# svg-project/Sparse-VideoGen

Measured on AMD Instinct MI355X. Metric: attn_tflops_svg1_block_sparse, higher is better.
Workload: dtype bf16; 1 GPU; HunyuanVideo T2V hy720p SVG1 sparse layer-call: sample_mse(64 rows) + band attention with fused head placement, cfg=1 H=24 D=128 F=33 P=3600 ctx=256 prompt=64 S=119056 band=15616 density=0.2456; parallelism=single, variant=0, heads=alt

## Files before the change

include/svg_attn.h:

```cpp
#ifndef SVG_ATTN_H_
#define SVG_ATTN_H_

#include <stddef.h>
#include <stdint.h>

#ifdef __cplusplus
extern "C" {
#endif

#define SVG_DTYPE_BF16 0
#define SVG_DTYPE_F16 1
#define SVG_DTYPE_F32 2

#define SVG_OK 0
#define SVG_ERR_BAD_ARG (-1)
#define SVG_ERR_UNSUPPORTED (-2)
#define SVG_ERR_WORKSPACE (-3)
#define SVG_ERR_LAUNCH (-4)

#define SVG_ABI_VERSION 4
int svg_abi_version(void);

const char* svg_strerror(int code);
int svg_last_hip_error(void);
// ... 239 lines not shown
                              float sm_scale, const svg_band_mask_t* masks, const svg_band_mask_t* alt_masks,
                              const int32_t* group_heads, int32_t n_groups, const svg_perm_desc_t* perm,
                              const int32_t* use_alt_flag, int32_t q_prescaled, const svg_attn_layout_t* layout, void* stream);

size_t svg_band_attention_fp8_workspace_bytes(int32_t BH, int32_t S, int32_t D);
int svg_band_attention_fp8(const void* q, const void* k, const void* v, void* o, int32_t BH, int32_t S, int32_t D, int32_t dtype,
                           float sm_scale, const svg_band_mask_t* mask, const svg_perm_desc_t* perm, void* workspace,
                           size_t workspace_bytes, void* stream);
int svg_band_attention_fp8_stage(const void* q, const void* k, const void* v, void* o, int32_t BH, int32_t S, int32_t D, int32_t dtype,
                                 float sm_scale, const svg_band_mask_t* mask, const svg_perm_desc_t* perm, void* workspace,
                                 size_t workspace_bytes, int32_t stage, void* stream);

size_t svg_varblock_attention_fp8_workspace_bytes(int32_t Hq, int32_t Hkv, int32_t QB, int32_t KB, int32_t Sq, int32_t Skv, int32_t D);
int svg_varblock_attention_fp8(const void* q, const void* k, const void* v, void* o, int32_t Hq, int32_t Hkv, int32_t Sq, int32_t Skv,
                               int32_t D, int32_t dtype, float sm_scale, const uint8_t* block_map, const int32_t* q_sizes,
                               const int32_t* k_sizes, int32_t QB, int32_t KB, const int32_t* q_row_idx, const int32_t* kv_row_idx,
                               void* workspace, size_t workspace_bytes, void* stream);

int32_t svg_band_attention_notify_target(int32_t S, const svg_band_mask_t* mask);
int svg_band_attention_notify(const void* q, const void* k, const void* v, void* o, int32_t BH, int32_t S, int32_t D,
                              int32_t dtype, float sm_scale, const svg_band_mask_t* mask, const svg_perm_desc_t* perm,
                              int32_t* done_per_head, int32_t done_words, void* stream);
int svg_wait_counters(const int32_t* counters, int32_t n, int32_t target, void* stream);
int svg_wait_counters_deadline(const int32_t* counters, int32_t n, int32_t target, int32_t timeout_ms, int32_t* timed_out,
                               void* stream);
int32_t svg_band_attention_notify_layout(int32_t S, const svg_band_mask_t* mask, int32_t nseg, int32_t* row_bounds, int32_t* targets);
int svg_band_attention_notify_seg(const void* q, const void* k, const void* v, void* o, int32_t BH, int32_t S, int32_t D,
                                  int32_t dtype, float sm_scale, const svg_band_mask_t* mask, const svg_perm_desc_t* perm,
                                  int32_t* done, int32_t done_words, int32_t nseg, void* stream);
int svg_band_attention_prescaled_notify_seg(const void* q_scaled, const void* k, const void* v, void* o, int32_t BH, int32_t S,
                                            int32_t D, int32_t dtype, const svg_band_mask_t* mask, const svg_perm_desc_t* perm,
                                            int32_t* done, int32_t done_words, int32_t nseg, void* stream);

int32_t svg_band_queue_order(int32_t BH, int32_t S, const svg_band_mask_t* mask, int32_t* out, int32_t out_words);
int svg_debug_band_queue_cap(int32_t max_workgroups);
int64_t svg_debug_band_replays(int32_t reset);
int32_t svg_debug_band_row_cursor(int32_t S, int32_t vid0, int32_t num_frame, int32_t frame_size, int32_t token_major,
                                  const int32_t* k0, int32_t n, int32_t* out, int32_t out_words, int32_t* cheap);

int svg_debug_pp_trace(uint64_t* out104);

int svg_debug_clock_probe(const int32_t* stop_flag, uint64_t* out2, int32_t max_ms, void* stream);

int svg_debug_wg_trace(uint64_t* out, int32_t n_workgroups);

#ifdef __cplusplus
}
#endif

#include "svg_attn_sparse_lse.h"
#include "svg_attn_f32_parts.h"
#include "svg_attn_band_lse_forms.h"
#include "svg_attn_band_window.h"
#include "svg_attn_band_shard.h"
#include "svg_attn_band_shard_switch.h"
#include "svg_attn_profile_shard.h"
#endif
```

sparse-videogen_amd/csrc/attention.hip:

```cpp
#include <algorithm>
#include <atomic>
#include <mutex>

#include "attn_core.h"
#include "attn_m16.h"
#include "band_policy.h"

namespace svg {

template <typename T, int D, int NW>
__global__ __launch_bounds__(NW * 64, 2) void band_attn_kernel(typename BandPolicy<T, D, NW>::Params prm) {
    extern __shared__ __attribute__((aligned(16))) char smem[];
    attn_body<T, D, NW, BandPolicy<T, D, NW>>(prm, smem, nullptr);
}

template <typename T, int D>
__global__ __launch_bounds__(512, (D == 64 ? 4 : 2)) void band_attn_pp2_kernel(typename BandPolicy<T, D, 8>::Params prm) {
    extern __shared__ __attribute__((aligned(16))) char smem[];
    attn_body_pp2<T, D, BandPolicy<T, D, 8>, false, 0, false, D == 64>(prm, smem, nullptr);
}
template <typename T>
__global__ __launch_bounds__(512, 4) void band_attn_pp2_switch64_kernel(typename BandPolicy<T, 64, 8>::Params prm,
                                                                        typename BandPolicy<T, 64, 8>::Params prm_alt,
                                                                        const int32_t* __restrict__ flag) {
// ... 912 lines not shown
extern "C" int64_t svg_debug_band_replays(int32_t reset) {
    unsigned n = 0;
    if (hipDeviceSynchronize() != hipSuccess || hipMemcpyFromSymbol(&n, HIP_SYMBOL(g_band_replays), sizeof n) != hipSuccess) return -1;
    const unsigned zero = 0;
    if (reset && hipMemcpyToSymbol(HIP_SYMBOL(g_band_replays), &zero, sizeof zero) != hipSuccess) return -1;
    return (int64_t)n;
}

extern "C" int32_t svg_debug_band_row_cursor(int32_t S, int32_t vid0, int32_t num_frame, int32_t frame_size, int32_t token_major,
                                             const int32_t* k0, int32_t n, int32_t* out, int32_t out_words, int32_t* cheap) {
    using Pol = svg::BandPolicy<__bf16, 128, 8>;
    if (S <= 0 || n < 0 || !k0 || !out || (int64_t)out_words < (int64_t)n * kBN) return -1;
    const svg_band_mask_t mask{S, S, 0, 0, 0, 0};
    const int64_t flag = 1;
    const svg_perm_desc_t perm{&flag, vid0, num_frame, frame_size};
    if (check_band_mask(S, &mask, &perm) != SVG_OK) return -1;
    const Pol::Params p = svg::make_band_params<Pol, __bf16>(nullptr, nullptr, nullptr, nullptr, 1, S, 1.f, &mask, &perm);
    Pol::Ctx c{};
    c.perm = token_major != 0;
    for (int row = 0; row < kBN; ++row) {
        Pol::RowWalk w;
        Pol::row_walk_init(p, c, w);
        int phys = 0;
        for (int i = 0; i < n; ++i) {
            Pol::RowWalk probe = w;
            if (cheap) cheap[i] = Pol::row_walk_cheap(probe, k0[i]) ? 1 : 0;
            Pol::row_walk_next(p, w, phys, k0[i], row);
            out[(size_t)i * kBN + row] = phys;
        }
    }
    return n;
}

extern "C" int svg_debug_wg_trace(uint64_t* out, int n_workgroups) { return g_trace_reader(out, true, n_workgroups); }
extern "C" int svg_debug_pp_trace(uint64_t* out104) { return g_trace_reader(out104, false, 0); }
```

sparse-videogen_amd/csrc/attn_m16.h:

```cpp
#pragma once
#include "attn_core.h"

namespace svg {

template <typename T>
struct Mfma16;
template <>
struct Mfma16<__bf16> {
    static __device__ __forceinline__ f32x4 mfma(bf16x8 a, bf16x8 b, f32x4 c) { return __builtin_amdgcn_mfma_f32_16x16x32_bf16(a, b, c, 0, 0, 0); }
    static __device__ __forceinline__ f32x4 mfma_keep_c(bf16x8 a, bf16x8 b, const f32x4& c) {
        f32x4 d;
        asm volatile("v_mfma_f32_16x16x32_bf16 %0, %1, %2, %3" : "=&v"(d) : "v"(a), "v"(b), "v"(c));
        return d;
    }
};
template <>
struct Mfma16<_Float16> {
    static __device__ __forceinline__ f32x4 mfma(f16x8 a, f16x8 b, f32x4 c) { return __builtin_amdgcn_mfma_f32_16x16x32_f16(a, b, c, 0, 0, 0); }
    static __device__ __forceinline__ f32x4 mfma_keep_c(f16x8 a, f16x8 b, const f32x4& c) {
        f32x4 d;
        asm volatile("v_mfma_f32_16x16x32_f16 %0, %1, %2, %3" : "=&v"(d) : "v"(a), "v"(b), "v"(c));
        return d;
    }
};
// ... 53 lines not shown
struct HasRowO32<P, std::void_t<decltype(&P::o32_base)>> : std::true_type {};
template <typename T, typename E>
__device__ __forceinline__ f32x4 o32_values(const f32x4& acc, float inv) {
    f32x4 o4;
    if constexpr (std::is_same_v<T, _Float16>) {
        typename E::v4 h4;
#pragma unroll
        for (int j = 0; j < 4; ++j) h4[j] = E::from_float(acc[j] * inv);
        u32x2 hb = __builtin_bit_cast(u32x2, h4);
        asm("" : "+v"(hb));
        h4 = __builtin_bit_cast(typename E::v4, hb);
#pragma unroll
        for (int j = 0; j < 4; ++j) {
            float a = acc[j];
            asm("" : "+v"(a));
            float p = a * inv;
            asm("" : "+v"(p));
            const float h = (float)h4[j];
            if ((float)(_Float16)p != h)
                p = __uint_as_float(fabsf(h) > fabsf(p) ? __float_as_uint(p) + 1u : __float_as_uint(p) - 1u);
            o4[j] = p;
        }
    } else {
#pragma unroll
        for (int j = 0; j < 4; ++j) o4[j] = acc[j] * inv;
    }
    return o4;
}

template <typename P, typename = void>
struct HasRowCursor : std::false_type {};
template <typename P>
struct HasRowCursor<P, std::void_t<decltype(P::kRowCursor)>> : std::true_type {};

template <bool when_set>
__device__ __forceinline__ void pp_barrier_sel(int flag) {
    __builtin_amdgcn_sched_barrier(0);
    if constexpr (when_set) asm volatile("s_cmp_eq_u32 %0, 0\n\ts_cbranch_scc1 1f\n\ts_waitcnt lgkmcnt(0)\n\ts_barrier\n1:" ::"s"(flag) : "memory", "scc");
    else asm volatile("s_cmp_lg_u32 %0, 0\n\ts_cbranch_scc1 1f\n\ts_waitcnt lgkmcnt(0)\n\ts_barrier\n1:" ::"s"(flag) : "memory", "scc");
    __builtin_amdgcn_sched_barrier(0);
}

template <typename T>
__device__ __forceinline__ u32x2 add_rounded16(u32x2 a, u32x2 b) {
    using E = Elt<T>;
    const typename E::v4 x = __builtin_bit_cast(typename E::v4, a), y = __builtin_bit_cast(typename E::v4, b);
    typename E::v4 s;
#pragma unroll
    for (int j = 0; j < 4; ++j) s[j] = E::from_float(E::to_float(x[j]) + E::to_float(y[j]));
    return __builtin_bit_cast(u32x2, s);
}

constexpr int kCheckEvery = 8;
template <typename T, typename P, bool TRACE = false, int ONEBAR = -1, bool PRE = false, bool SPEC = false>
__device__ __forceinline__ bool attn_m16_tile(const typename P::Params& prm, const typename P::Ctx& ctx, char* smem,
                                              int check_mask = kCheckEvery - 1, unsigned* replay_ctr = nullptr) {
    using E = Elt<T>;
    using M = Mfma16<T>;
    using V8 = typename E::v8;
    constexpr int D = 128;
    constexpr int NW = 8;
    constexpr int KS = D / 32;
    constexpr int NDB = D / 16;
    using Img = KvImage16<D>;
    constexpr int NS = 4;
    constexpr int kImg = Img::kImg, kStage = Img::kStage;
// ... 44 lines not shown
    int nphys = 0, nnext = 0;
    unsigned req_ko = 0, req_vo = 0;
    auto resolve = [&](int t, auto guard_c) {
        if constexpr (kCursor) {
            if (!decltype(guard_c)::value || t < nT) P::row_walk_next(prm, cur, nnext, P::tile_key0(ctx, t), krow);
        } else if constexpr (decltype(guard_c)::value) {
            nnext = (t < nT) ? P::kv_phys(prm, ctx, cur, t, krow) : 0;
        } else {
            nnext = P::kv_phys(prm, ctx, cur, t, krow);
        }
    };
    constexpr std::true_type kGuarded{};
    auto take = [&]() {
        if constexpr (kCursor) {
            req_ko = __umul24((unsigned)nnext, k_rsb) + col_v;
            req_vo = __umul24((unsigned)nnext, v_rsb) + col_v;
            asm volatile("" : "+v"(req_ko), "+v"(req_vo));
        } else {
            nphys = nnext;
        }
    };
    auto dma_piece = [&](int t, auto j_c) {
        constexpr int j = decltype(j_c)::value;
        const unsigned st = __builtin_amdgcn_readfirstlane(lds_piece + (unsigned)((t % NS) * kStage) + j * (kBN * 64));
        const unsigned ko = kCursor ? req_ko : __umul24((unsigned)nphys, k_rsb) + col_v;
        const unsigned vo = kCursor ? req_vo : __umul24((unsigned)nphys, v_rsb) + col_v;
        lds_dma16_kv<kImg>(st, ko, vo, (const char*)kb_ + j * 64, (const char*)vb + j * 64);
    };
    auto dma_issue = [&](int t) {
        dma_piece(t, std::integral_constant<int, 0>{});
        dma_piece(t, std::integral_constant<int, 1>{});
    };
    const int dist = lagging ? 3 : 2;
    for (int t = 0; t < dist; ++t) {
        resolve(t, kGuarded);
        take();
        if (t < nT) dma_issue(t);
    }
    resolve(dist, kGuarded);

    int q_log[2];
    V8 qf[2][KS];
    int m_a0[2], m_b0[2];
    unsigned m_alen[2], m_blen[2];
#pragma unroll
    for (int rb = 0; rb < 2; ++rb) {
        const int row_in_wg = wave * 32 + rb * 16 + n16;
        const int qp = P::q_phys(prm, ctx, row_in_wg);
        q_log[rb] = P::q_logical(ctx, row_in_wg);
        const T* qrow = qb + (size_t)(qp >= 0 ? qp : 0) * P::q_rs(prm) + g4 * 8;
#pragma unroll
        for (int ks = 0; ks < KS; ++ks) qf[rb][ks] = *(const V8*)(qrow + ks * 32);
        P::row_intervals(prm, ctx, q_log[rb], m_a0[rb], m_alen[rb], m_b0[rb], m_blen[rb]);
    }

    const int k_lane = Img::k_lane(g4, n16);
    const int v_lane0 = Img::v_lane0(g4, n16);
    const int v_lane1 = v_lane0 ^ 32;

    float m_run[2] = {-INFINITY, -INFINITY}, m_use[2] = {0.f, 0.f}, l_run[2] = {0.f, 0.f}, psum[2] = {0.f, 0.f};
    float m_sub[2] = {kBias, kBias};
    f32x4 acc_l[2] = {{0.f, 0.f, 0.f, 0.f}, {0.f, 0.f, 0.f, 0.f}};
    V8 ones8;
#pragma unroll
    for (int j = 0; j < 8; ++j) ones8[j] = E::from_float(1.f);
    bool force_exact = true;
// ... 37 lines not shown
    float psum_thr = -1.f;

    auto kfrag = [&](const char* st, int kblk, int ks) -> i16x8 { return Img::kfrag(st, k_lane, kblk, ks); };
    auto vfrag = [&](const char* st, int kc, int db) -> i16x8 { return Img::vfrag(st, v_lane0, v_lane1, kc, db); };
    auto probs_impl = [&](int kc, auto shifted_c) {
        constexpr bool shifted = decltype(shifted_c)::value;
#pragma unroll
        for (int rb = 0; rb < 2; ++rb)
#pragma unroll
            for (int h = 0; h < 2; ++h)
#pragma unroll
                for (int r = 0; r < 4; ++r) {
                    float p;
                    if constexpr (PRE && shifted) p = __builtin_amdgcn_exp2f(sc[2 * kc + h][rb][r] + pre_shift[rb]);
                    else if constexpr (PRE) p = __builtin_amdgcn_exp2f(sc[2 * kc + h][rb][r]);
                    else p = __builtin_amdgcn_exp2f(__builtin_fmaf(sc[2 * kc + h][rb][r], c_log2, -m_sub[rb]));
                    if constexpr (!MSUM) psum[rb] += p;
                    pf[kc][rb][4 * h + r] = E::from_float(p);
                }
    };
    auto probs = [&](int kc) { probs_impl(kc, std::false_type{}); };
    auto stage_resolve_next = [&](int t, auto guard_c) {
        take();
        resolve(t + dist + 1, guard_c);
    };
    auto stage_request = [&](int t) {
        const bool more = t + dist < nT;
        if (more) dma_issue(t + dist);
        if (more) asm volatile("s_waitcnt vmcnt(%0)" ::"n"(2 * NP) : "memory");
        else asm volatile("s_waitcnt vmcnt(0)" ::: "memory");
    };
    auto vector_phase = [&](int t, auto guard_c) {
        constexpr bool guard = decltype(guard_c)::value;
        stage_resolve_next(t, guard_c);
        const bool more = !guard || t + dist < nT;
        if (more) dma_piece(t + dist, std::integral_constant<int, 0>{});
        const int tk0 = P::tile_key0(ctx, t);
        const int cls = P::classify(prm, ctx, tk0, wave * 32);
        if (cls != TILE_FULL) {
            const bool part = (cls == TILE_PARTIAL);
#pragma unroll
            for (int rb = 0; rb < 2; ++rb) {
                int ka = tk0 + 4 * g4 - m_a0[rb], kb2 = tk0 + 4 * g4 - m_b0[rb];
                asm volatile("" : "+v"(ka), "+v"(kb2));
#pragma unroll
                for (int b = 0; b < 4; ++b)
#pragma unroll
                    for (int r = 0; r < 4; ++r) {
                        const int key = 16 * b + r;
                        const bool ok = ((unsigned)(ka + key) < m_alen[rb]) | ((unsigned)(kb2 + key) < m_blen[rb]);
                        sc[b][rb][r] = (part & ok) ? sc[b][rb][r] : -INFINITY;
                    }
            }
        }
        if (more) dma_piece(t + dist, std::integral_constant<int, 1>{});
        psum[0] = 0.f, psum[1] = 0.f;
#pragma unroll
        for (int kc = 0; kc < 2; ++kc) {
            probs(kc);
            asm volatile("" : "+v"(pf[kc][0]), "+v"(pf[kc][1]), "+v"(psum[0]), "+v"(psum[1]));
        }
        bool exact;
        if constexpr (MSUM) {
            typedef unsigned u32x4_t __attribute__((ext_vector_type(4)));
            const u32x4_t w0 = __builtin_bit_cast(u32x4_t, pf[0][0]), w1 = __builtin_bit_cast(u32x4_t, pf[0][1]);
            const u32x4_t w2 = __builtin_bit_cast(u32x4_t, pf[1][0]), w3 = __builtin_bit_cast(u32x4_t, pf[1][1]);
            const unsigned o0 = w0[0] | w0[1] | w0[2], o1 = w0[3] | w1[0] | w1[1], o2 = w1[2] | w1[3] | w2[0];
            const unsigned o3 = w2[1] | w2[2] | w2[3], o4 = w3[0] | w3[1] | w3[2];
            if constexpr (kSpec) {
                exact = spec_mode < 0;
                if (spec_mode >= 0 && (t & spec_mode) == 0) {
// ... 310 lines not shown
```

sparse-videogen_amd/csrc/band_policy.h:

```cpp
#pragma once
#include <algorithm>

#include "attn_core.h"

namespace svg {

struct BandOpts {
    int32_t* done = nullptr;
    int done_nseg = 1;
    bool prescaled = false;
    bool trace = false;
    int trace_abl = 0;
    bool strided = false;
    AttnLayout lay{};
    const svg_band_mask_t* alt_mask = nullptr;
    const int32_t* use_alt = nullptr;
    float* lse = nullptr;
    float* o32 = nullptr;
    const svg_band_shard_t* q_shard = nullptr;
    const svg_band_shard_t* k_shard = nullptr;
};

inline int check_band_mask(int S, const svg_band_mask_t* mask, const svg_perm_desc_t* perm) {
    if (mask->real_len < 0 || mask->real_len > S || mask->band < 0 || mask->band > S + 1) return SVG_ERR_BAD_ARG;
// ... 59 lines not shown
        }
        return logical;
    }

    static __device__ __forceinline__ bool init(const Params& p, Ctx& c, char*) {
        int qt;
        const int nh = p.BH * p.n_heavy;
        const int b = blockIdx.x;
        if (b >= p.nqt * p.BH) return false;
        if (b < nh) {
            c.head = b / p.n_heavy;
            qt = p.heavy_lo + (b - c.head * p.n_heavy);
        } else {
            const int b2 = b - nh;
            const int full = ((p.nqt * p.BH - nh) / (kNumXCD * 32)) * (kNumXCD * 32);
            int w2 = b2;
            if (b2 < full) {
                const int xcd = b2 % kNumXCD, s = b2 / kNumXCD;
                w2 = (s / 32) * (kNumXCD * 32) + xcd * 32 + (s % 32);
            }
            const int nl = p.nqt - p.n_heavy;
            c.head = w2 / nl;
            const int r = w2 - c.head * nl;
            qt = r < p.heavy_lo ? r : r + p.n_heavy;
        }
        init_tile(p, c, c.head, qt);
        return true;
    }

    static __device__ __forceinline__ void init_tile(const Params& p, Ctx& c, int head, int qt) {
        c.head = head;
        c.perm = (p.head_flag != nullptr) && (p.head_flag[c.head] != 0);
        kv_schedule(p, c, qt);
        const int real = p.real_len;
        const int w0 = c.q0 + wave_id() * kWR, w1 = min(w0 + kWR, c.q_end);
        c.fk_lo = 1, c.fk_hi = 0;
        if (w0 < c.q_end && w1 <= real) {
            const bool full_rows = w0 >= p.rf_lo && w1 <= p.rf_hi;
            c.fk_lo = full_rows ? 0 : max(w1 - p.band, 0);
            c.fk_hi = min(full_rows ? real : w0 + p.band - kBN, min(real, p.S) - kBN);
        }
    }

    static __host__ __device__ __forceinline__ void kv_schedule(const Params& p, Ctx& c, int qt) {
        using std::max;
        using std::min;
        const bool r1 = qt >= p.reg_t0[1], r2 = qt >= p.reg_t0[2], r3 = qt >= p.reg_t0[3];
        const int rlo = r3 ? p.reg_lo[3] : r2 ? p.reg_lo[2] : r1 ? p.reg_lo[1] : p.reg_lo[0];
        const int rhi = r3 ? p.reg_hi[3] : r2 ? p.reg_hi[2] : r1 ? p.reg_hi[1] : p.reg_hi[0];
        const int rt0 = r3 ? p.reg_t0[3] : r2 ? p.reg_t0[2] : r1 ? p.reg_t0[1] : 0;
        c.qt = qt;
        c.q0 = rlo + (qt - rt0) * BM;
        c.q_end = min(rhi, c.q0 + BM);

        constexpr int BIG = 1 << 28;
        int alo = BIG, ahi = BIG, blo = BIG, bhi = BIG, clo = BIG, chi = BIG;
        const int real = p.real_len;
        if (c.q0 < real) {
            const int qr1 = min(c.q_end, real);
            if (c.q0 < p.rf_hi && qr1 > p.rf_lo) {
                alo = 0, ahi = (real + kBN - 1) / kBN;
            } else {
                alo = max(0, c.q0 - p.band + 1) / kBN;
                ahi = (min(real, qr1 - 1 + p.band) + kBN - 1) / kBN;
                const int ch = min(p.cf_hi, real);
                if (ch > p.cf_lo) blo = p.cf_lo / kBN, bhi = (ch + kBN - 1) / kBN;
            }
        }
        if (c.q_end > real) clo = real / kBN, chi = (p.S + kBN - 1) / kBN;
#define SVG_CSWAP(x, xh, y, yh) if (y < x) { int t_ = x; x = y; y = t_; t_ = xh; xh = yh; yh = t_; }
        SVG_CSWAP(alo, ahi, blo, bhi)
        SVG_CSWAP(blo, bhi, clo, chi)
        SVG_CSWAP(alo, ahi, blo, bhi)
#undef SVG_CSWAP
        if (blo < BIG && blo <= ahi) {
            ahi = max(ahi, bhi);
            blo = clo, bhi = chi, clo = BIG, chi = BIG;
            if (blo < BIG && blo <= ahi) ahi = max(ahi, bhi), blo = BIG, bhi = BIG;
        } else if (clo < BIG && clo <= bhi) {
            bhi = max(bhi, chi), clo = BIG, chi = BIG;
        }
        c.seg_lo[0] = alo, c.seg_n[0] = ahi - alo;
        c.seg_lo[1] = blo, c.seg_n[1] = bhi - blo;
        c.seg_lo[2] = clo, c.seg_n[2] = chi - clo;
        c.nT = c.seg_n[0] + c.seg_n[1] + c.seg_n[2];
    }

    static __device__ __forceinline__ int q_logical(const Ctx& c, int row) { return c.q0 + row; }
    static __device__ __forceinline__ bool wave_active(const Ctx& c, int wrow0) { return c.q0 + wrow0 < c.q_end; }
    static __device__ __forceinline__ int q_phys(const Params& p, const Ctx& c, int row) {
        const int l = c.q0 + row;
        return l < c.q_end ? phys_row(p, c, l) : -1;
    }
    static __device__ __forceinline__ int tile_key0(const Ctx& c, int t) {
        const int n01 = c.seg_n[0] + c.seg_n[1];
        const int a = c.seg_lo[0] + t, b = c.seg_lo[1] + (t - c.seg_n[0]), d = c.seg_lo[2] + (t - n01);
        const int bd = t < n01 ? b : d;
        return (t < c.seg_n[0] ? a : bd) * kBN;
    }
    struct TileCur {
        int k0, left;
        int k1, left1;
        int k2, left2;
    };
    static __device__ __forceinline__ void tile_cur_shift(TileCur& tc) {
        tc.k0 = tc.k1, tc.left = tc.left1;
        tc.k1 = tc.k2, tc.left1 = tc.left2;
        tc.left2 = 0;
    }
    static __device__ __forceinline__ void tile_cur_init(const Ctx& c, TileCur& tc) {
        tc.k0 = c.seg_lo[0] * kBN, tc.left = c.seg_n[0];
        tc.k1 = c.seg_lo[1] * kBN, tc.left1 = c.seg_n[1];
        tc.k2 = c.seg_lo[2] * kBN, tc.left2 = c.seg_n[2];
        if (tc.left <= 0) tile_cur_shift(tc);
        if (tc.left <= 0) tile_cur_shift(tc);
    }
    static __device__ __forceinline__ void tile_cur_next(const Ctx& c, TileCur& tc) {
        tile_cur_step(tc);
        if (tile_cur_ended(tc)) tile_cur_fix(c, tc);
    }
    static __device__ __forceinline__ void tile_cur_step(TileCur& tc) {
        tc.k0 += kBN;
        --tc.left;
    }
    static __device__ __forceinline__ bool tile_cur_ended(const TileCur& tc) { return tc.left <= 0; }
    static __device__ __forceinline__ void tile_cur_fix(const Ctx&, TileCur& tc) {
        tile_cur_shift(tc);
        if (tc.left <= 0) tile_cur_shift(tc);
    }
    static constexpr bool kRowStep = true;
    struct RowState {
        int l, f, physv;
    };
    static __device__ __forceinline__ void rows_seek(const Params& p, const Ctx& c, RowState& st, int k0, int row) {
        st.l = k0 + row;
        const int i = st.l - p.vid0;
        const int a = i >= 0 ? i : -i - 1;
        const int qd = (int)((unsigned)a / (unsigned)p.F);
        const int pp = i >= 0 ? qd : -qd - 1;
        st.f = i - pp * p.F;
        st.physv = p.vid0 + st.f * p.P + pp;
    }
    static __device__ __forceinline__ void rows_step(const Params& p, const Ctx&, RowState& st) {
        st.l += kBN;
        int f = st.f + p.r64, physv = st.physv + p.sp64;
        const bool wrap = f >= p.F;
        st.f = wrap ? f - p.F : f;
        st.physv = wrap ? physv + p.wrap_phys : physv;
    }
    static __device__ __forceinline__ int rows_phys(const Params& p, const Ctx& c, const RowState& st) {
        const bool in_video = (unsigned)(st.l - p.vid0) < (unsigned)p.V;
        const int phys = (c.perm && in_video) ? st.physv : st.l;
        return st.l < p.S ? phys : 0;
    }
    static __device__ __forceinline__ bool fast_full(const Ctx& c, int k0) { return k0 >= c.fk_lo && k0 <= c.fk_hi; }
    static __device__ __forceinline__ void kv_cursor_init(const Params&, const Ctx&, KvCursor& cu, int) {
        cu.physv = 0, cu.f = 0, cu.prev_k0 = -(1 << 30);
    }
    static __device__ __forceinline__ int kv_phys(const Params& p, const Ctx& c, KvCursor& cu, int t, int row) {
        return kv_phys_at(p, c, cu, tile_key0(c, t), row);
    }
    static __device__ __forceinline__ int kv_phys_at(const Params& p, const Ctx& c, KvCursor& cu, int k0, int row) {
        const int l = k0 + row;
        if (!c.perm) return l < p.S ? l : 0;
        int f, physv;
        const int delta = __builtin_amdgcn_readfirstlane(k0 - cu.prev_k0);
        if (delta == kBN) {
            f = cu.f + p.r64;
            physv = cu.physv + p.sp64;
            const bool wrap = f >= p.F;
            f = wrap ? f - p.F : f;
            physv = wrap ? physv + p.wrap_phys : physv;
        } else {
            const int i = l - p.vid0;
            const int a = i >= 0 ? i : -i - 1;
            const int qd = (int)((unsigned)a / (unsigned)p.F);
            const int pp = i >= 0 ? qd : -qd - 1;
            f = i - pp * p.F;
            physv = p.vid0 + f * p.P + pp;
        }
        cu.physv = physv, cu.f = f, cu.prev_k0 = k0;
        if (k0 >= p.vid0 && k0 + kBN <= p.vid0 + p.V) return physv;
        const bool in_video = (unsigned)(l - p.vid0) < (unsigned)p.V;
        const int phys = in_video ? physv : l;
        return l < p.S ? phys : 0;
    }

    static constexpr bool kRowCursor = true;
// ... 19 lines not shown
    }
    static __host__ __device__ __forceinline__ bool row_walk_cheap(RowWalk& w, int k0) {
        const bool cheap = (k0 == w.prev_k0 + kBN) & (k0 >= w.lo) & (k0 <= w.hi);
        w.prev_k0 = k0;
        return cheap;
    }
    static __host__ __device__ __forceinline__ void row_add(int& phys, int d) {
#ifdef __HIP_DEVICE_COMPILE__
        asm("v_add_u32 %0, %0, %1" : "+v"(phys) : "v"(d));
#else
        phys += d;
#endif
    }
    static __host__ __device__ __forceinline__ void row_set(int& phys, int x) {
#ifdef __HIP_DEVICE_COMPILE__
        asm("v_mov_b32 %0, %1" : "+v"(phys) : "v"(x));
#else
        phys = x;
#endif
    }
    static __host__ __device__ __forceinline__ int row_exact(const Params& p, int vlen, int l) {
        const int i = l - p.vid0;
        const int a = i >= 0 ? i : -i - 1;
        const int qd = (int)((unsigned)a / (unsigned)p.F);
        const int pp = i >= 0 ? qd : -qd - 1;
        const int f = i - pp * p.F;
        const int physv = p.vid0 + f * p.P + pp;
        const bool in_video = (unsigned)i < (unsigned)vlen;
        const int phys = in_video ? physv : l;
        return l < p.S ? phys : 0;
    }
    static __host__ __device__ __forceinline__ void row_walk_next(const Params& p, RowWalk& w, int& phys, int k0, int row) {
        const bool cheap = row_walk_cheap(w, k0);
        row_add(phys, w.step);
        if (w.perm) row_add(phys, phys >= w.end ? w.unwrap : 0);
        if (__builtin_expect(!cheap, 0)) row_set(phys, row_exact(p, w.vlen, k0 + row));
    }

    static __device__ __forceinline__ int classify(const Params& p, const Ctx& c, int k0, int wrow0) {
        if (k0 >= c.fk_lo && k0 <= c.fk_hi) return TILE_FULL;
        const int w0 = c.q0 + wrow0;
        if (w0 >= c.q_end) return TILE_SKIP;
        const int w1 = min(w0 + kWR, c.q_end);
        const int k1 = min(k0 + kBN, p.S);
        const int real = p.real_len;
        bool all = false;
        if (k0 + kBN <= p.S) {
            if (w1 <= real && k1 <= real) {
                const bool band_all = (k1 - 1 - w0 < p.band) && (w1 - 1 - k0 < p.band);
                const bool col_all = (k0 >= p.cf_lo && k1 <= p.cf_hi);
                const bool row_all = (w0 >= p.rf_lo && w1 <= p.rf_hi);
                all = band_all || col_all || row_all;
            } else if (w0 >= real && k0 >= real) {
                all = true;
            }
        }
        if (all) return TILE_FULL;
        bool any = false;
        if (w0 < real && k0 < real) {
            const int w1r = min(w1, real), k1r = min(k1, real);
            const bool band_any = (k0 - (w1r - 1) < p.band) && (w0 - (k1r - 1) < p.band);
            const bool col_any = (k0 < p.cf_hi && k1r > p.cf_lo);
            const bool row_any = (w0 < p.rf_hi && w1r > p.rf_lo);
            any = band_any || col_any || row_any;
        }
        if (w1 > real && k1 > real) any = true;
        return any ? TILE_PARTIAL : TILE_SKIP;
    }
    static __device__ __forceinline__ bool allowed(const Params& p, const Ctx&, int q, int k) {
// ... 31 lines not shown
                        const int t_hi = (sgm == p.done_nseg - 1) ? p.nqt : min(p.nqt, (sgm + 1) * p.done_tps);
                        atomicAdd(cnt + sgm, (t_hi - t_lo) * NW);
                    }
                }
            }
        }
    }
};

template <typename T>
struct BandLsePolicy : BandPolicy<T, 128, 8> {
    using Base = BandPolicy<T, 128, 8>;
    struct Params : Base::Params {
        float* lse;
    };
    static __device__ __forceinline__ float* lse_base(const Params& p, const typename Base::Ctx& c) { return p.lse + (size_t)c.head * (size_t)p.S; }
};

template <typename T>
struct BandF32Policy : BandLsePolicy<T> {
    using Base = BandLsePolicy<T>;
    struct Params : Base::Params {
        float* o32;
    };
    static __device__ __forceinline__ float* o32_base(const Params& p, const typename Base::Ctx& c) {
        return p.o32 + (size_t)c.head * (size_t)p.S * 128;
    }
};

template <typename BasePol>
struct BandWindowOf : BasePol {
    using Ctx = typename BasePol::Ctx;
    using RowWalk = typename BasePol::RowWalk;
    struct Params : BasePol::Params {
        int q_begin, Sq;
        int k_begin, k_end;
    };
    static __host__ __device__ __forceinline__ void clip_keys(const Params& p, Ctx& c) {
        using std::max;
        using std::min;
        const int t_lo = p.k_begin / kBN, t_hi = (p.k_end + kBN - 1) / kBN;
#define SVG_CLIP_SEG(i)                                                                  \
    {                                                                                    \
        const int lo = max(c.seg_lo[i], t_lo), hi = min(c.seg_lo[i] + c.seg_n[i], t_hi); \
        c.seg_lo[i] = lo, c.seg_n[i] = max(hi - lo, 0);                                  \
    }
        SVG_CLIP_SEG(0) SVG_CLIP_SEG(1) SVG_CLIP_SEG(2)
#undef SVG_CLIP_SEG
        c.nT = c.seg_n[0] + c.seg_n[1] + c.seg_n[2];
    }
    static __host__ __device__ __forceinline__ void kv_schedule(const Params& p, Ctx& c, int qt) {
        BasePol::kv_schedule(p, c, qt);
        clip_keys(p, c);
    }
    static __device__ __forceinline__ void init_tile(const Params& p, Ctx& c, int head, int qt) {
        BasePol::init_tile(p, c, head, qt);
        clip_keys(p, c);
        c.fk_hi = min(c.fk_hi, p.k_end - kBN);
    }
    static __device__ __forceinline__ bool init(const Params& p, Ctx& c, char* lds) {
        if (!BasePol::init(p, c, lds)) return false;
        clip_keys(p, c);
        c.fk_hi = min(c.fk_hi, p.k_end - kBN);
        return true;
    }
    static __device__ __forceinline__ int q_phys(const Params& p, const Ctx& c, int row) {
// ... 30 lines not shown
    static __device__ __forceinline__ float* o32_base(const typename Base::Params& p, const typename Base::Ctx& c) {
        return p.o32 + (size_t)c.head * (size_t)p.Sq * 128;
    }
};

struct BandShardMap {
    int f0, Fl, nv, n, tail_begin;
    int fdiv;
    int sp64;
    __host__ __device__ __forceinline__ int g(int vid0, int F, int P, int kind, int l) const {
        const int pp = (int)((unsigned)l / (unsigned)fdiv), fl = l - pp * fdiv;
        const int gv = kind ? vid0 + pp * F + f0 + fl : vid0 + f0 * P + l;
        return l < nv ? gv : tail_begin + (l - nv);
    }
    __host__ __device__ __forceinline__ int ginv(int vid0, int F, int P, int kind, int x) const {
        using std::max;
        using std::min;
        const int y = x - vid0, yc = max(y, 0);
        const int pp = (int)((unsigned)yc / (unsigned)F), r = yc - pp * F;
        const int l1 = pp * Fl + min(max(r - f0, 0), Fl);
        const int lv = min(kind ? l1 : max(y - f0 * P, 0), nv);
        const int lt = nv + min(max(x - tail_begin, 0), n - nv);
        return lv < nv ? lv : lt;
    }
    __host__ __device__ __forceinline__ int phys(int P, int kind, int l) const {
        const int pp = (int)((unsigned)l / (unsigned)fdiv), fl = l - pp * fdiv;
        return (kind && l < nv) ? fl * P + pp : l;
    }
};

template <typename BasePol>
struct BandShardOf : BasePol {
    using RowWalk = typename BasePol::RowWalk;
    struct Ctx : BasePol::Ctx {
        int gw0, gw1;
    };
    struct Params : BasePol::Params {
        BandShardMap qs, ks;
        int reg1_lo[4], reg1_hi[4], reg1_t0[4];
    };
    static __device__ __forceinline__ int gq(const Params& p, const Ctx& c, int l) { return p.qs.g(p.vid0, p.F, p.P, c.perm, l); }
    static __device__ __forceinline__ int gk(const Params& p, const Ctx& c, int l) { return p.ks.g(p.vid0, p.F, p.P, c.perm, l); }
    static __device__ __forceinline__ int ginv_k(const Params& p, const Ctx& c, int x) { return p.ks.ginv(p.vid0, p.F, p.P, c.perm, x); }

    static __device__ __forceinline__ void kv_schedule(const Params& p, Ctx& c, int qt) {
        const bool k1 = c.perm != 0;
#define SVG_REG(a, i) (k1 ? p.reg1_##a[i] : p.reg_##a[i])
        const bool r1 = qt >= SVG_REG(t0, 1), r2 = qt >= SVG_REG(t0, 2), r3 = qt >= SVG_REG(t0, 3);
        const int rlo = r3 ? SVG_REG(lo, 3) : r2 ? SVG_REG(lo, 2) : r1 ? SVG_REG(lo, 1) : SVG_REG(lo, 0);
        const int rhi = r3 ? SVG_REG(hi, 3) : r2 ? SVG_REG(hi, 2) : r1 ? SVG_REG(hi, 1) : SVG_REG(hi, 0);
        const int rt0 = r3 ? SVG_REG(t0, 3) : r2 ? SVG_REG(t0, 2) : r1 ? SVG_REG(t0, 1) : 0;
#undef SVG_REG
        c.qt = qt;
        c.q0 = rlo + (qt - rt0) * BasePol::BM;
        c.q_end = min(rhi, c.q0 + BasePol::BM);
        constexpr int BIG = 1 << 28;
        int alo = BIG, ahi = BIG, blo = BIG, bhi = BIG, clo = BIG, chi = BIG;
        if (c.q0 < c.q_end) {
            const int g0 = gq(p, c, c.q0), g1 = gq(p, c, c.q_end - 1) + 1;
            const int real = p.real_len;
            auto tiles = [&](int a, int b, int& lo, int& hi) {
                const int x = ginv_k(p, c, a), y = ginv_k(p, c, b);
                if (b > a && y <= x) return;
                lo = x / kBN, hi = max((y + kBN - 1) / kBN, lo);
            };
            if (g0 < real) {
// ... 344 lines not shown
```

sparse-videogen_amd/svg/_native.py:

```python
from __future__ import annotations

import ctypes as C
import os
from pathlib import Path
from typing import NamedTuple, Optional, Sequence

import torch

_LIB_PATH = Path(__file__).resolve().parent.parent / "lib" / "libsvgattn.so"
_lib: Optional[C.CDLL] = None
_load_error: Optional[str] = None

SVG_DTYPE_BF16, SVG_DTYPE_F16 = 0, 1


POISON_BYTE = 0xFF


def poison_storage(t: torch.Tensor) -> torch.Tensor:
    st = t.untyped_storage()
    if st.nbytes():
        torch.zeros(0, dtype=torch.uint8, device=t.device).set_(st).fill_(POISON_BYTE)
    return t

# ... 66 lines not shown
        ("emulate_bf16", C.c_int32),
        ("variant", ProfileVariant * 2),
    ]


_I32, _I64, _F32, _VP, _SZ = C.c_int32, C.c_int64, C.c_float, C.c_void_p, C.c_size_t


class PrologueSegment(C.Structure):
    _fields_ = [("q_in", C.c_void_p), ("k_in", C.c_void_p), ("v_in", C.c_void_p), ("rows", C.c_int32), ("norm_kind", C.c_int32),
                ("q_weight", C.c_void_p), ("q_bias", C.c_void_p), ("k_weight", C.c_void_p), ("k_bias", C.c_void_p), ("eps", C.c_float)]


class TensorStrides(C.Structure):
    _fields_ = [("batch", C.c_int64), ("head", C.c_int64), ("row", C.c_int64)]


class AttnLayout(C.Structure):
    _fields_ = [("heads_per_batch", C.c_int32), ("kv_heads_per_batch", C.c_int32), ("q", TensorStrides), ("k", TensorStrides),
                ("v", TensorStrides), ("o", TensorStrides)]


SIGNATURES = {
    "svg_abi_version": (C.c_int, []),
    "svg_strerror": (C.c_char_p, [C.c_int]),
    "svg_last_hip_error": (C.c_int, []),
    "svg_build_info": (C.c_char_p, []),
    "svg_debug_pp_trace": (C.c_int, [_VP]),
    "svg_debug_wg_trace": (C.c_int, [_VP, _I32]),
    "svg_band_queue_order": (_I32, [_I32, _I32, C.POINTER(BandMask), _VP, _I32]),
    "svg_debug_band_queue_cap": (C.c_int, [_I32]),
    "svg_debug_band_replays": (C.c_int64, [_I32]),
    "svg_debug_band_row_cursor": (_I32, [_I32, _I32, _I32, _I32, _I32, _VP, _I32, _VP, _I32, _VP]),
    "svg_rms_norm_forward": (C.c_int, [_VP, _VP, C.c_int64, _I32, _I32, C.c_float, _VP]),
    "svg_layer_norm_forward": (C.c_int, [_VP, _VP, _VP, C.c_int64, _I32, _I32, _VP]),
    "svg_apply_qk_rope_inplace_cossin": (C.c_int, [_VP, _VP, _VP, _VP, _I32, _I32, _I32, _I32, _I32, _I32, _I32, _VP]),
    "svg_apply_qk_rope_inplace_cossin_txtlast": (C.c_int, [_VP, _VP, _VP, _VP, _I32, _I32, _I32, _I32, _I32, _I32, _I32, _VP]),
    "svg_apply_qk_rope_inplace_cossin_complex": (C.c_int, [_VP, _VP, _VP, _VP, _I32, _I32, _I32, _I32, _I32, _I32, _I32, _VP]),
    "svg_bsr_to_block_map": (C.c_int, [_VP, _VP, _I32, _I32, _I32, _I32, _I32, _I32, _VP, _VP, _VP, _VP]),
    "svg_layernorm_forward": (C.c_int, [_VP, _VP, _VP, _VP, C.c_int64, _I32, _I32, _I32, _I32, C.c_float, _VP]),
    "svg_rmsnorm_forward": (C.c_int, [_VP, _VP, _VP, C.c_int64, _I32, _I32, _I32, _I32, C.c_float, _VP]),
    "svg_layernorm_forward_ex": (C.c_int, [_VP, _VP, _VP, _VP, C.c_int64, _I32, _I32, _I32, _I32, C.c_float, _I32, _VP]),
    "svg_modulate_shift_forward": (C.c_int, [_VP, _VP, _VP, _VP, C.c_int64, _I32, C.c_int64, _I32, _I32, _VP]),
    "svg_modulate_gate_residual_forward": (C.c_int, [_VP, _VP, _VP, _VP, C.c_int64, _I32, C.c_int64, _I32, _I32, _I32, _VP]),
    "svg_layernorm_modulate_forward": (C.c_int, [_VP, _VP, _VP, _VP, _VP, _VP, C.c_int64, _I32, C.c_int64, _I32, _I32, _I32,
                                                 C.c_float, _VP]),
    "svg_layernorm_modulate_forward_ex": (C.c_int, [_VP, _VP, _VP, _VP, _VP, _VP, C.c_int64, _I32, C.c_int64, _I32, _I32, _I32,
                                                    C.c_float, _I32, _VP]),
    "svg_qk_norm_rope_transpose": (C.c_int, [_VP, _VP, _VP, _VP, _I32, _I32, _I32, _I32, _I32, _I32, _I32, _VP, _VP, _VP, _VP,
                                             C.c_float, _I32, _VP, _VP, _I32, _I32, _VP]),
    "svg_qk_norm_rope": (C.c_int, [_VP, _VP, _I32, _I32, _I32, _I32, _I32, _I32, _I32, _VP, _VP, _VP, _VP, C.c_float, _I32, _VP,
                                   _VP, _I32, _I32, _VP]),
    "svg_qk_norm_rope_qscale": (C.c_int, [_VP, _VP, _I32, _I32, _I32, _I32, _I32, _I32, _I32, _VP, _VP, _VP, _VP, C.c_float, _I32, _VP,
                                          _VP, _I32, _I32, C.c_float, _VP]),
    "svg_qk_norm_rope_transpose_qscale": (C.c_int, [_VP, _VP, _VP, _VP, _I32, _I32, _I32, _I32, _I32, _I32, _I32, _VP, _VP, _VP, _VP,
                                                    C.c_float, _I32, _VP, _VP, _I32, _I32, C.c_float, _VP]),
    "svg_qk_norm_rope_transpose_joint": (C.c_int, [C.POINTER(PrologueSegment), _I32, _VP, _VP, _VP, _I32, _I32, _I32, _I32, _I32, _VP, _VP,
                                                   _I32, _I32, C.c_float, _VP]),
    "svg_rmsnorm_rope_transpose": (C.c_int, [_VP, _VP, _VP, _VP, _VP, _VP, _I32, _I32, _I32, _I32, _I32, _VP, _VP, _I32, C.c_float, _I32, _VP,
                                             _VP, _I32, _I32, C.c_float, _VP]),
    "svg_head_placement": (C.c_int, [_VP, _VP, _I32, _VP, _I32, _I32, _I32, _I32, _I32, _I32, _I32, _I32, _I32, _VP]),
    "svg_permute_rows": (C.c_int, [_VP, _VP, _VP, _I32, _I32, _I32, _I32, _VP]),
    "svg_inverse_permute_rows": (C.c_int, [_VP, _VP, _VP, _I32, _I32, _I32, _I32, _VP]),
    "svg_argsort_workspace_bytes": (_SZ, [_I32, _I32, _I32]),
    "svg_argsort_labels": (C.c_int, [_VP, _VP, _VP, _I32, _I32, _I32, _VP, _SZ, _VP]),
    "svg_band_attention": (C.c_int, [_VP, _VP, _VP, _VP, _I32, _I32, _I32, _I32, _F32, C.POINTER(BandMask),
# ... 1813 lines not shown
```

Before: 1350 TFLOP/s.

## Precompute contiguous fast tile run to skip per-tile cursor checks and classify

Before the main loop, each wave computes the longest run of tiles that are contiguous and fully inside the band's fast interval. Inside that run, the vector phase skips the row-cursor cheap/exact check, the tile key lookup and the tile classification, and just advances the cursor by a fixed step. This cuts scalar and vector bookkeeping per KV tile in the band attention hot loop. A host-visible debug entry point is added to check the run bounds and row addresses against the exact walk. The risk is wrong addressing or masking if the run bounds are computed incorrectly.

```diff
diff --git a/include/svg_attn.h b/include/svg_attn.h
--- a/include/svg_attn.h
+++ b/include/svg_attn.h
@@ -295,6 +295,9 @@
                                             int32_t D, int32_t dtype, const svg_band_mask_t* mask, const svg_perm_desc_t* perm,
                                             int32_t* done, int32_t done_words, int32_t nseg, void* stream);
 
+int32_t svg_debug_band_tile_run(int32_t S, const svg_band_mask_t* mask, int32_t vid0, int32_t num_frame, int32_t frame_size,
+                                int32_t token_major, int32_t qt, int32_t wave, int32_t dist, int32_t* out4, int32_t* tiles,
+                                int32_t tiles_words, int32_t* rows, int32_t rows_words);
 int32_t svg_band_queue_order(int32_t BH, int32_t S, const svg_band_mask_t* mask, int32_t* out, int32_t out_words);
 int svg_debug_band_queue_cap(int32_t max_workgroups);
 int64_t svg_debug_band_replays(int32_t reset);
diff --git a/sparse-videogen_amd/csrc/attention.hip b/sparse-videogen_amd/csrc/attention.hip
--- a/sparse-videogen_amd/csrc/attention.hip
+++ b/sparse-videogen_amd/csrc/attention.hip
@@ -968,5 +968,65 @@
     return n;
 }
 
+extern "C" int32_t svg_debug_band_tile_run(int32_t S, const svg_band_mask_t* mask, int32_t vid0, int32_t num_frame, int32_t frame_size,
+                                           int32_t token_major, int32_t qt, int32_t wave, int32_t dist, int32_t* out4, int32_t* tiles,
+                                           int32_t tiles_words, int32_t* rows, int32_t rows_words) {
+    using Pol = svg::BandPolicy<__bf16, 128, 8>;
+    if (S <= 0 || !mask || !out4 || wave < 0 || wave >= 8 || dist < 1 || dist > 8 || qt < 0) return -1;
+    if (num_frame <= 0 && token_major) return -1;
+    const int64_t flag = 1;
+    const svg_perm_desc_t perm{&flag, vid0, num_frame, frame_size};
+    const svg_perm_desc_t* pd = num_frame > 0 ? &perm : nullptr;
+    if (check_band_mask(S, mask, pd) != SVG_OK) return -1;
+    const Pol::Params p = svg::make_band_params<Pol, __bf16>(nullptr, nullptr, nullptr, nullptr, 1, S, 1.f, mask, pd);
+    if (qt >= p.nqt) return -1;
+    Pol::Ctx c{};
+    c.perm = token_major != 0;
+    Pol::kv_schedule(p, c, qt);
+    Pol::wave_fast_interval(p, c, wave, c.fk_lo, c.fk_hi);
+    const int nT = c.nT;
+    if ((tiles && (int64_t)tiles_words < (int64_t)nT * 4) || (rows && (int64_t)rows_words < (int64_t)nT * kBN)) return -1;
+    Pol::RowWalk w0;
+    Pol::row_walk_init(p, c, w0);
+    int run_lo = 0, run_n = 0;
+    Pol::tile_run(c, w0, dist, run_lo, run_n);
+    out4[0] = run_lo, out4[1] = run_n, out4[2] = nT, out4[3] = p.nqt;
+    if (tiles) {
+        for (int t = 0; t < nT; ++t) {
+            const int k0 = Pol::tile_key0(c, t);
+            tiles[4 * t] = k0;
+            tiles[4 * t + 1] = Pol::fast_full(c, k0) ? 1 : 0;
+            tiles[4 * t + 2] = (t > 0 && k0 == Pol::tile_key0(c, t - 1) + kBN) ? 1 : 0;
+            int cheap = 0;
+            if (t + dist + 1 < nT) {
+                Pol::RowWalk probe = w0;
+                probe.prev_k0 = Pol::tile_key0(c, t + dist);
+                cheap = Pol::row_walk_cheap(probe, Pol::tile_key0(c, t + dist + 1)) ? 1 : 0;
+            }
+            tiles[4 * t + 3] = cheap;
+        }
+    }
+    if (rows) {
+        for (int row = 0; row < kBN; ++row) {
+            Pol::RowWalk w = w0;
+            int phys = 0;
+            for (int t = 0; t <= dist && t < nT; ++t) {
+                Pol::row_walk_next(p, w, phys, Pol::tile_key0(c, t), row);
+                rows[(size_t)t * kBN + row] = phys;
+            }
+            for (int t = 0; t + dist + 1 < nT; ++t) {
+                Pol::row_walk_step(w, phys);
+                if ((unsigned)(t - run_lo) < (unsigned)run_n) Pol::row_walk_in_run(w);
+                else {
+                    const int k_next = Pol::tile_key0(c, t + dist + 1);
+                    if (!Pol::row_walk_cheap(w, k_next)) Pol::row_walk_exact(p, w, phys, k_next, row);
+                }
+                rows[(size_t)(t + dist + 1) * kBN + row] = phys;
+            }
+        }
+    }
+    return nT;
+}
+
 extern "C" int svg_debug_wg_trace(uint64_t* out, int n_workgroups) { return g_trace_reader(out, true, n_workgroups); }
 extern "C" int svg_debug_pp_trace(uint64_t* out104) { return g_trace_reader(out104, false, 0); }
diff --git a/sparse-videogen_amd/csrc/attn_m16.h b/sparse-videogen_amd/csrc/attn_m16.h
--- a/sparse-videogen_amd/csrc/attn_m16.h
+++ b/sparse-videogen_amd/csrc/attn_m16.h
@@ -109,6 +109,28 @@
 struct HasRowCursor : std::false_type {};
 template <typename P>
 struct HasRowCursor<P, std::void_t<decltype(P::kRowCursor)>> : std::true_type {};
+
+template <typename P, typename = void>
+struct HasTileRun : std::false_type {};
+template <typename P>
+struct HasTileRun<P, std::enable_if_t<P::kTileRun>> : std::true_type {};
+template <typename P, bool = HasTileRun<P>::value>
+struct TileRunOps {
+    template <typename... A> static __device__ __forceinline__ void step(A&...) {}
+    template <typename... A> static __device__ __forceinline__ void in_run(A&...) {}
+    template <typename... A> static __device__ __forceinline__ bool cheap(A&...) { return true; }
+    template <typename... A> static __device__ __forceinline__ void exact(A&...) {}
+};
+template <typename P>
+struct TileRunOps<P, true> {
+    using W = typename P::RowWalk;
+    static __device__ __forceinline__ void step(const W& w, int& phys) { P::row_walk_step(w, phys); }
+    static __device__ __forceinline__ void in_run(W& w) { P::row_walk_in_run(w); }
+    static __device__ __forceinline__ bool cheap(W& w, const int& k0) { return P::row_walk_cheap(w, k0); }
+    static __device__ __forceinline__ void exact(const typename P::Params& p, const W& w, int& phys, const int& k0, const int& row) {
+        P::row_walk_exact(p, w, phys, k0, row);
+    }
+};
 
 template <bool when_set>
 __device__ __forceinline__ void pp_barrier_sel(int flag) {
@@ -219,6 +241,12 @@
         dma_piece(t, std::integral_constant<int, 1>{});
     };
     const int dist = lagging ? 3 : 2;
+    constexpr bool kRun = kCursor && HasTileRun<P>::value;
+    int run_lo = 0, run_n = 0;
+    if constexpr (kRun) {
+        P::tile_run(ctx, cur, dist, run_lo, run_n);
+        run_lo = __builtin_amdgcn_readfirstlane(run_lo), run_n = __builtin_amdgcn_readfirstlane(run_n);
+    }
     for (int t = 0; t < dist; ++t) {
         resolve(t, kGuarded);
         take();
@@ -322,11 +350,34 @@
     };
     auto vector_phase = [&](int t, auto guard_c) {
         constexpr bool guard = decltype(guard_c)::value;
-        stage_resolve_next(t, guard_c);
+        constexpr bool run_form = kRun && !guard;
+        int tk0 = 0, cls = TILE_FULL;
+        if constexpr (run_form) {
+            using R = TileRunOps<P>;
+            const bool in_run = (unsigned)(t - run_lo) < (unsigned)run_n;
+            take();
+            R::step(cur, nnext);
+            dma_piece(t + dist, std::integral_constant<int, 0>{});
+            bool cheap = true;
+            int k_next = 0;
+            if (__builtin_expect(in_run, 1)) {
+                R::in_run(cur);
+            } else {
+                k_next = P::tile_key0(ctx, t + dist + 1);
+                cheap = R::cheap(cur, k_next);
+                tk0 = P::tile_key0(ctx, t);
+                cls = P::classify(prm, ctx, tk0, wave * 32);
+            }
+            if (__builtin_expect(!cheap, 0)) R::exact(prm, cur, nnext, k_next, krow);
+        } else {
+            stage_resolve_next(t, guard_c);
+        }
         const bool more = !guard || t + dist < nT;
-        if (more) dma_piece(t + dist, std::integral_constant<int, 0>{});
-        const int tk0 = P::tile_key0(ctx, t);
-        const int cls = P::classify(prm, ctx, tk0, wave * 32);
+        if constexpr (!run_form) {
+            if (more) dma_piece(t + dist, std::integral_constant<int, 0>{});
+            tk0 = P::tile_key0(ctx, t);
+            cls = P::classify(prm, ctx, tk0, wave * 32);
+        }
         if (cls != TILE_FULL) {
             const bool part = (cls == TILE_PARTIAL);
 #pragma unroll
diff --git a/sparse-videogen_amd/csrc/band_policy.h b/sparse-videogen_amd/csrc/band_policy.h
--- a/sparse-videogen_amd/csrc/band_policy.h
+++ b/sparse-videogen_amd/csrc/band_policy.h
@@ -115,13 +115,20 @@
         c.head = head;
         c.perm = (p.head_flag != nullptr) && (p.head_flag[c.head] != 0);
         kv_schedule(p, c, qt);
+        wave_fast_interval(p, c, wave_id(), c.fk_lo, c.fk_hi);
+    }
+    static __host__ __device__ __forceinline__ void wave_fast_interval(const Params& p, const Ctx& c, int wave, int& lo, int& hi) {
+#ifndef __HIP_DEVICE_COMPILE__
+        using std::max;
+        using std::min;
+#endif
         const int real = p.real_len;
-        const int w0 = c.q0 + wave_id() * kWR, w1 = min(w0 + kWR, c.q_end);
-        c.fk_lo = 1, c.fk_hi = 0;
+        const int w0 = c.q0 + wave * kWR, w1 = min(w0 + kWR, c.q_end);
+        lo = 1, hi = 0;
         if (w0 < c.q_end && w1 <= real) {
             const bool full_rows = w0 >= p.rf_lo && w1 <= p.rf_hi;
-            c.fk_lo = full_rows ? 0 : max(w1 - p.band, 0);
-            c.fk_hi = min(full_rows ? real : w0 + p.band - kBN, min(real, p.S) - kBN);
+            lo = full_rows ? 0 : max(w1 - p.band, 0);
+            hi = min(full_rows ? real : w0 + p.band - kBN, min(real, p.S) - kBN);
         }
     }
 
@@ -175,7 +182,7 @@
         const int l = c.q0 + row;
         return l < c.q_end ? phys_row(p, c, l) : -1;
     }
-    static __device__ __forceinline__ int tile_key0(const Ctx& c, int t) {
+    static __host__ __device__ __forceinline__ int tile_key0(const Ctx& c, int t) {
         const int n01 = c.seg_n[0] + c.seg_n[1];
         const int a = c.seg_lo[0] + t, b = c.seg_lo[1] + (t - c.seg_n[0]), d = c.seg_lo[2] + (t - n01);
         const int bd = t < n01 ? b : d;
@@ -236,7 +243,7 @@
         const int phys = (c.perm && in_video) ? st.physv : st.l;
         return st.l < p.S ? phys : 0;
     }
-    static __device__ __forceinline__ bool fast_full(const Ctx& c, int k0) { return k0 >= c.fk_lo && k0 <= c.fk_hi; }
+    static __host__ __device__ __forceinline__ bool fast_full(const Ctx& c, int k0) { return k0 >= c.fk_lo && k0 <= c.fk_hi; }
     static __device__ __forceinline__ void kv_cursor_init(const Params&, const Ctx&, KvCursor& cu, int) {
         cu.physv = 0, cu.f = 0, cu.prev_k0 = -(1 << 30);
     }
@@ -322,9 +329,40 @@
     }
     static __host__ __device__ __forceinline__ void row_walk_next(const Params& p, RowWalk& w, int& phys, int k0, int row) {
         const bool cheap = row_walk_cheap(w, k0);
+        row_walk_step(w, phys);
+        if (__builtin_expect(!cheap, 0)) row_set(phys, row_exact(p, w.vlen, k0 + row));
+    }
+    static __host__ __device__ __forceinline__ void row_walk_step(const RowWalk& w, int& phys) {
         row_add(phys, w.step);
         if (w.perm) row_add(phys, phys >= w.end ? w.unwrap : 0);
-        if (__builtin_expect(!cheap, 0)) row_set(phys, row_exact(p, w.vlen, k0 + row));
+    }
+    static __host__ __device__ __forceinline__ void row_walk_exact(const Params& p, const RowWalk& w, int& phys, int k0, int row) {
+        row_set(phys, row_exact(p, w.vlen, k0 + row));
+    }
+    static __host__ __device__ __forceinline__ void row_walk_in_run(RowWalk& w) { w.prev_k0 += kBN; }
+
+    static constexpr bool kTileRun = true;
+    static __host__ __device__ __forceinline__ void tile_run(const Ctx& c, const RowWalk& w, int dist, int& run_lo, int& run_n) {
+        using std::max;
+        using std::min;
+        static_assert(kBN == 64, "tile_run divides by the tile size with a shift");
+        run_lo = 0, run_n = 0;
+        const int ahead = (dist + 1) * kBN;
+        const int k_lo = max(c.fk_lo, w.lo - ahead), k_hi = min(c.fk_hi, w.hi - ahead);
+        int t0 = 0;
+#define SVG_RUN_SEG(i)                                                                         \
+    {                                                                                          \
+        const int n = c.seg_n[i];                                                              \
+        if (n > dist + 2) {                                                                    \
+            const int kf = c.seg_lo[i] * kBN;                                                  \
+            const int j_lo = max(1, (k_lo - kf + kBN - 1) >> 6);                               \
+            const int j_hi = min(n - dist - 2, (k_hi - kf) >> 6);                              \
+            if (j_hi - j_lo + 1 > run_n) run_lo = t0 + j_lo, run_n = j_hi - j_lo + 1;          \
+        }                                                                                      \
+        t0 += n;                                                                               \
+    }
+        SVG_RUN_SEG(0) SVG_RUN_SEG(1) SVG_RUN_SEG(2)
+#undef SVG_RUN_SEG
     }
 
     static __device__ __forceinline__ int classify(const Params& p, const Ctx& c, int k0, int wrow0) {
@@ -422,6 +460,7 @@
 struct BandWindowOf : BasePol {
     using Ctx = typename BasePol::Ctx;
     using RowWalk = typename BasePol::RowWalk;
+    static constexpr bool kTileRun = false;
     struct Params : BasePol::Params {
         int q_begin, Sq;
         int k_begin, k_end;
@@ -518,6 +557,7 @@
 template <typename BasePol>
 struct BandShardOf : BasePol {
     using RowWalk = typename BasePol::RowWalk;
+    static constexpr bool kTileRun = false;
     struct Ctx : BasePol::Ctx {
         int gw0, gw1;
     };
diff --git a/sparse-videogen_amd/svg/_native.py b/sparse-videogen_amd/svg/_native.py
--- a/sparse-videogen_amd/svg/_native.py
+++ b/sparse-videogen_amd/svg/_native.py
@@ -122,6 +122,7 @@
     "svg_debug_band_queue_cap": (C.c_int, [_I32]),
     "svg_debug_band_replays": (C.c_int64, [_I32]),
     "svg_debug_band_row_cursor": (_I32, [_I32, _I32, _I32, _I32, _I32, _VP, _I32, _VP, _I32, _VP]),
+    "svg_debug_band_tile_run": (_I32, [_I32, C.POINTER(BandMask), _I32, _I32, _I32, _I32, _I32, _I32, _I32, _VP, _VP, _I32, _VP, _I32]),
     "svg_rms_norm_forward": (C.c_int, [_VP, _VP, C.c_int64, _I32, _I32, C.c_float, _VP]),
     "svg_layer_norm_forward": (C.c_int, [_VP, _VP, _VP, C.c_int64, _I32, _I32, _VP]),
     "svg_apply_qk_rope_inplace_cossin": (C.c_int, [_VP, _VP, _VP, _VP, _I32, _I32, _I32, _I32, _I32, _I32, _I32, _VP]),
```

New measurement: 1375 TFLOP/s (median of 6 runs). +1.8%, better.
